# lucidrains/DALLE-pytorch

Measured on AMD Instinct MI355X. Metric: img-tokens/sec, higher is better.
Workload: dtype bf16; 1 GPU; model=dalle-dim1024-depth12-heads16, reversible=True, global_batch=64, seq_len=1280, image_seq_len=1024, parallelism=dp1, mode=train, eager=False

## Files before the change

dalle_pytorch_amd/ops/fp8.py:

```python

import weakref

import torch
import torch.nn.functional as F

from dalle_pytorch_amd.ops.dispatch import (env_flag, hip_module,
                                            using_eager_fallback)
from dalle_pytorch_amd.ops.fused import (fusion_enabled, geglu_bwd_colsum,
                                         geglu_colsum_tiles)

_FORCED = None
FP8_MAX = 448.0


def set_fp8_enabled(flag):
    global _FORCED
    _FORCED = bool(flag) if flag is not None else None


def fp8_enabled():
    if _FORCED is not None:
        return _FORCED
    return env_flag('FP8', False)


_generation = 0


def fp8_mark_step():
    global _generation
    _generation += 1


class _StepCache:

    BOUND = 512

    def __init__(self, make):
        self.make = make
        self.entries = {}

    def __call__(self, w):
        key = (w.data_ptr(), tuple(w.shape))
        stamp = (w._version, _generation)
        owner = w._base if w._base is not None else w
        hit = self.entries.get(key)
        if hit is not None and hit[0] == stamp and hit[2]() is owner:
            return hit[1]
        val = self.make(w)
        if len(self.entries) >= self.BOUND:
            self.entries.clear()
        self.entries[key] = (stamp, val, weakref.ref(owner))
        return val


def _bf16(w):
    w = w.detach()
    return w if w.dtype == torch.bfloat16 else w.to(torch.bfloat16)


def _quant(t, ext):
    t = t.detach().contiguous()
    scale = ext.amax_bf16(t)
    return ext.quant_fp8(t, scale), scale.squeeze()


_quant_weight = _StepCache(lambda w: _quant(_bf16(w), hip_module()))
_bf16_weight = _StepCache(_bf16)
_transposed_weight = _StepCache(lambda w: _bf16(w).t().contiguous())


def _fp8_ok(x, weight):
    if not fp8_enabled() or using_eager_fallback(x):
        return False
    if x.dtype != torch.bfloat16:
        return False
    rows = x.numel() // x.shape[-1]
    k, n = weight.shape[1], weight.shape[0]
    if rows % 16 or k % 16 or n % 16 or rows < 256:
        return False
    if rows * k < (32 << 20):
        return False
    return n * 2 >= k * 3


def _fast_dgrad_ok(x, w):
    if using_eager_fallback(x) or x.dtype != torch.bfloat16:
        return False
    rows = x.numel() // x.shape[-1]
    return (rows >= 1024 and rows % 16 == 0 and w.shape[0] % 16 == 0
            and w.shape[1] % 16 == 0 and torch.is_grad_enabled())


def _gemm_forward(x, weight, bias):
    x2 = x.reshape(-1, x.shape[-1])
    if _fp8_ok(x, weight):
        xq, xs = _quant(x2, hip_module())
        wq, ws = _quant_weight(weight)
        out = torch._scaled_mm(xq, wq.t(), scale_a=xs, scale_b=ws,
                               bias=bias, out_dtype=torch.bfloat16)
    else:
        wb = weight if weight.dtype == torch.bfloat16 else _bf16_weight(weight)
        out = F.linear(x, wb, bias).reshape(-1, weight.shape[0])
    return x2, out


def _gemm_backward(do2, x2, weight, lead):
    wt = _transposed_weight(weight)
    dx = (do2 @ wt.t()).reshape(*lead, weight.shape[1])
    dw = do2.t() @ x2.to(do2.dtype)
    return dx, dw.to(weight.dtype)


def _bf16_bias(bias):
    if bias is None or bias.dtype == torch.bfloat16:
        return bias
    return bias.to(torch.bfloat16)


class _LinearFn(torch.autograd.Function):

    @staticmethod
    def forward(ctx, x, weight, bias):
        x2, out = _gemm_forward(x, weight, _bf16_bias(bias))
        ctx.save_for_backward(x2, weight)
        ctx.has_bias = bias is not None
        return out.reshape(*x.shape[:-1], weight.shape[0])

    @staticmethod
    def backward(ctx, dout):
        x2, weight = ctx.saved_tensors
        do2 = dout.reshape(-1, dout.shape[-1]).contiguous()
        dx, dw = _gemm_backward(do2, x2, weight, dout.shape[:-1])
        return dx, dw, do2.sum(0) if ctx.has_bias else None


def fp8_linear_raw(x, weight, bias, module=None):
    if (_fp8_ok(x, weight) or _fast_dgrad_ok(x, weight)) \
            and weight.is_contiguous():
        return _LinearFn.apply(x.contiguous(), weight, bias)
    return F.linear(x, weight, bias) if module is None else module(x)


def fp8_linear(linear_module, x):
    return fp8_linear_raw(x, linear_module.weight, linear_module.bias,
                          linear_module)


class _LinearGegluFn(torch.autograd.Function):

    @staticmethod
    def forward(ctx, x, weight, bias):
        x2, h = _gemm_forward(x, weight, _bf16_bias(bias))
        out = hip_module().geglu_fwd(h)
        ctx.save_for_backward(x2, weight, h)
        ctx.bias_dtype = bias.dtype
        return out.reshape(*x.shape[:-1], weight.shape[0] // 2)

    @staticmethod
    def backward(ctx, dout):
        x2, weight, h = ctx.saved_tensors
        do2 = dout.reshape(-1, dout.shape[-1]).contiguous()
        dh, db = geglu_bwd_colsum(h, do2)
        dx, dw = _gemm_backward(dh, x2, weight, dout.shape[:-1])
        return dx, dw, db.to(ctx.bias_dtype)


def linear_geglu_ok(linear_module, x):
    w = linear_module.weight
    return (fusion_enabled('FF1_BIAS') and linear_module.bias is not None
            and (_fp8_ok(x, w) or _fast_dgrad_ok(x, w))
            and geglu_colsum_tiles(w.shape[0]))


def linear_geglu(linear_module, x):
    return _LinearGegluFn.apply(x.contiguous(), linear_module.weight,
                                linear_module.bias)
```

dalle_pytorch_amd/ops/hip/build.py:

```python

import os
import subprocess
import sys
import sysconfig
import time
from concurrent.futures import ThreadPoolExecutor
from pathlib import Path

PKG_DIR = Path(__file__).resolve().parents[2]
SRC_DIR = Path(__file__).resolve().parent
SOURCES = [SRC_DIR / name for name in (
    'attention.hip', 'decode.hip', 'train_ops.hip', 'module.hip')]
OBJ_DIR = SRC_DIR / 'build'
OUTPUT = PKG_DIR / '_hip.so'
MAX_JOBS = 16


def _mtime(path):
    return path.stat().st_mtime if path.exists() else 0.0


def toolchain():
    import torch
    from torch.utils import cpp_extension as ce

    hipcc = str(Path(ce.ROCM_HOME or '/opt/rocm') / 'bin' / 'hipcc')
    abi = '1' if torch._C._GLIBCXX_USE_CXX11_ABI else '0'
    inc = [f'-I{p}' for p in ce.include_paths()]
    inc.append(f"-I{sysconfig.get_paths()['include']}")
    flags = [
        '-O3', '-std=c++17', '--offload-arch=gfx950',
        '-fPIC',
        '-DTORCH_EXTENSION_NAME=_hip',
        '-DTORCH_API_INCLUDE_EXTENSION_H',
        f'-D_GLIBCXX_USE_CXX11_ABI={abi}',
        *ce.COMMON_HIP_FLAGS, *ce.COMMON_HIPCC_FLAGS,
        '-DTORCH_HIP_VERSION=' + torch.version.hip.split('.')[0],
        '-Wno-deprecated-declarations', '-Wno-unused-result',
        *inc,
    ]
    return hipcc, flags, [f'-L{p}' for p in ce.library_paths()]


def build(verbose=True, force=False):
    newest_hdr = max((_mtime(h) for h in SRC_DIR.glob('*.h')), default=0.0)
    newest_src = max(newest_hdr, *(_mtime(s) for s in SOURCES))
    if not force and _mtime(OUTPUT) > newest_src:
        if verbose:
            print(f'[build] {OUTPUT.name} up to date')
        return str(OUTPUT)
    objs = [OBJ_DIR / (s.stem + '.o') for s in SOURCES]
    stale = [(s, o) for s, o in zip(SOURCES, objs)
             if force or _mtime(o) <= max(_mtime(s), newest_hdr)]

    hipcc, flags, libdirs = toolchain()

    def compile_unit(pair):
        src, obj = pair
        tmp = obj.with_suffix('.tmp.o')
        cmd = [hipcc, *flags, '-c', str(src), '-o', str(tmp)]
        if verbose:
            print('[build]', ' '.join(cmd), flush=True)
        t0 = time.time()
        res = subprocess.run(cmd, stdout=subprocess.PIPE,
                             stderr=subprocess.STDOUT, text=True)
        if res.returncode == 0:
            tmp.replace(obj)
        return src.name, res, time.time() - t0

    if stale:
        OBJ_DIR.mkdir(exist_ok=True)
        jobs = min(len(stale), MAX_JOBS, os.cpu_count() or 1)
        with ThreadPoolExecutor(max_workers=jobs) as pool:
            results = list(pool.map(compile_unit, stale))
        for name, res, secs in results:
            if verbose or res.returncode != 0:
                print(f'[build] {name}: exit {res.returncode}, {secs:.0f} s\n'
                      f'{res.stdout}', end='', flush=True)
        failed = [name for name, res, _ in results if res.returncode != 0]
        if failed:
            raise RuntimeError('hipcc failed for ' + ', '.join(failed))

    cmd = [
        hipcc, '--offload-arch=gfx950', '-fPIC', '-shared',
        *[str(o) for o in objs], *libdirs,
        '-ltorch', '-ltorch_cpu', '-ltorch_hip', '-lc10', '-lc10_hip',
        '-ltorch_python', '-lamdhip64',
        '-o', str(OUTPUT),
    ]
    if verbose:
        print('[build]', ' '.join(cmd), flush=True)
    subprocess.run(cmd, check=True)
    return str(OUTPUT)


if __name__ == '__main__':
    build(force='--force' in sys.argv)
```

Measured before the change: 305,400 img_tokens_per_sec.

## Add split-K weight-gradient GEMM with fp32 partials and fused reduce kernel

Adds a split-K path for the linear-layer weight gradient. The long row dimension (tokens) is cut into S power-of-two chunks and run as a batched GEMM into fp32 partials. A custom HIP kernel then sums the partials and casts them to the weight dtype. The aim is to fill the GPU's many compute units when the weight's n×k output has too few tiles for the GEMM to use them all. The cost is extra memory traffic and workspace for the S fp32 partial matrices, plus one more kernel launch per linear backward.

```diff
diff --git a/dalle_pytorch_amd/ops/fp8.py b/dalle_pytorch_amd/ops/fp8.py
--- a/dalle_pytorch_amd/ops/fp8.py
+++ b/dalle_pytorch_amd/ops/fp8.py
@@ -105,11 +105,51 @@
     return x2, out
 
 
+WGRAD_TILE = 256
+WGRAD_TILE_TARGET = 192
+WGRAD_ROW_FLOOR = 16384
+WGRAD_CHUNK_FLOOR = 5120
+WGRAD_MAX_SPLITS = 32
+
+
+def wgrad_splits(rows, n, k):
+    if rows < WGRAD_ROW_FLOOR or n <= 0 or k <= 0 or n % 16 or k % 16:
+        return 1
+    tiles = -(-n // WGRAD_TILE) * -(-k // WGRAD_TILE)
+    s = 1
+    while (s * tiles < WGRAD_TILE_TARGET and s < WGRAD_MAX_SPLITS
+           and rows % (2 * s) == 0 and rows // (2 * s) >= WGRAD_CHUNK_FLOOR):
+        s *= 2
+    return s
+
+
+def wgrad_plan(do2, x2, out_dtype):
+    s = wgrad_splits(do2.shape[0], do2.shape[-1], x2.shape[-1])
+    if s <= 1:
+        return 0
+    if not fusion_enabled('WGRAD_SPLITK') or using_eager_fallback(do2):
+        return 0
+    if not (do2.dtype == x2.dtype == torch.bfloat16 and do2.dim() == 2
+            and x2.dim() == 2 and do2.is_contiguous() and x2.is_contiguous()
+            and out_dtype in (torch.float32, torch.bfloat16)):
+        return 0
+    return s
+
+
+def _wgrad_op(do2, x2, splits, out_dtype):
+    return torch.ops.dalle_amd.wgrad_splitk(do2, x2, splits, out_dtype)
+
+
 def _gemm_backward(do2, x2, weight, lead):
     wt = _transposed_weight(weight)
     dx = (do2 @ wt.t()).reshape(*lead, weight.shape[1])
-    dw = do2.t() @ x2.to(do2.dtype)
-    return dx, dw.to(weight.dtype)
+    x2 = x2.to(do2.dtype)
+    splits = wgrad_plan(do2, x2, weight.dtype)
+    if splits:
+        dw = _wgrad_op(do2, x2, splits, weight.dtype)
+    else:
+        dw = (do2.t() @ x2).to(weight.dtype)
+    return dx, dw
 
 
 def _bf16_bias(bias):
diff --git a/dalle_pytorch_amd/ops/hip/build.py b/dalle_pytorch_amd/ops/hip/build.py
--- a/dalle_pytorch_amd/ops/hip/build.py
+++ b/dalle_pytorch_amd/ops/hip/build.py
@@ -10,7 +10,8 @@
 PKG_DIR = Path(__file__).resolve().parents[2]
 SRC_DIR = Path(__file__).resolve().parent
 SOURCES = [SRC_DIR / name for name in (
-    'attention.hip', 'decode.hip', 'train_ops.hip', 'module.hip')]
+    'attention.hip', 'decode.hip', 'train_ops.hip', 'wgrad.hip',
+    'module.hip')]
 OBJ_DIR = SRC_DIR / 'build'
 OUTPUT = PKG_DIR / '_hip.so'
 MAX_JOBS = 16
diff --git a/dalle_pytorch_amd/ops/hip/wgrad.hip b/dalle_pytorch_amd/ops/hip/wgrad.hip
--- /dev/null
+++ b/dalle_pytorch_amd/ops/hip/wgrad.hip
@@ -0,0 +1,120 @@
+
+#include <torch/library.h>
+
+#include "hip_host.h"
+
+
+template <int S, bool OUT_BF16>
+__global__ __launch_bounds__(256)
+void wgrad_reduce_kernel(const f32x4* __restrict__ part,
+                         void* __restrict__ out,
+                         long nvec) {
+  for (long i = (long)blockIdx.x * 256 + threadIdx.x; i < nvec;
+       i += (long)gridDim.x * 256) {
+    f32x4 v[S];
+    #pragma unroll
+    for (int s = 0; s < S; ++s) v[s] = part[(long)s * nvec + i];
+    f32x4 acc = v[0];
+    #pragma unroll
+    for (int s = 1; s < S; ++s) acc += v[s];
+    if (OUT_BF16) {
+      bf16x4 o;
+      #pragma unroll
+      for (int e = 0; e < 4; ++e) o[e] = f2bf(acc[e]);
+      reinterpret_cast<bf16x4*>(out)[i] = o;
+    } else {
+      reinterpret_cast<f32x4*>(out)[i] = acc;
+    }
+  }
+}
+
+constexpr int WGRAD_MAX_SPLITS = 32;
+
+static bool wgrad_dtype_ok(at::ScalarType t) {
+  return t == at::kFloat || t == at::kBFloat16;
+}
+
+template <int S>
+static void launch_reduce(const torch::Tensor& part, torch::Tensor& out) {
+  const long nvec = out.numel() / 4;
+  const long nb = std::max<long>(std::min<long>((nvec + 255) / 256, 2048), 1);
+  auto* p = reinterpret_cast<const f32x4*>(part.data_ptr<float>());
+  if (out.scalar_type() == at::kBFloat16)
+    hipLaunchKernelGGL((wgrad_reduce_kernel<S, true>), dim3(nb), dim3(256), 0,
+                       cur_stream(), p, out.data_ptr(), nvec);
+  else
+    hipLaunchKernelGGL((wgrad_reduce_kernel<S, false>), dim3(nb), dim3(256),
+                       0, cur_stream(), p, out.data_ptr(), nvec);
+}
+
+torch::Tensor wgrad_reduce(const torch::Tensor& part,
+                           at::ScalarType out_dtype) {
+  TORCH_CHECK(part.is_cuda() && part.dim() == 3 && part.is_contiguous(),
+              "wgrad_reduce: partials must be a contiguous [S, n, k] GPU "
+              "tensor");
+  TORCH_CHECK(part.scalar_type() == at::kFloat && wgrad_dtype_ok(out_dtype),
+              "wgrad_reduce: partials must be float32, the output float32 or "
+              "bfloat16");
+  const long S = part.size(0), n = part.size(1), k = part.size(2);
+  TORCH_CHECK(n * k > 0 && (n * k) % 4 == 0,
+              "wgrad_reduce: n * k must be a positive multiple of 4, got ", n,
+              " x ", k);
+  auto out = at::empty({n, k}, part.options().dtype(out_dtype));
+  switch (S) {
+    case 1: launch_reduce<1>(part, out); break;
+    case 2: launch_reduce<2>(part, out); break;
+    case 4: launch_reduce<4>(part, out); break;
+    case 8: launch_reduce<8>(part, out); break;
+    case 16: launch_reduce<16>(part, out); break;
+    case 32: launch_reduce<32>(part, out); break;
+    default:
+      TORCH_CHECK(false, "wgrad_reduce: S must be a power of two <= ",
+                  WGRAD_MAX_SPLITS, ", got ", S);
+  }
+  return out;
+}
+
+torch::Tensor wgrad_splitk(const torch::Tensor& do2, const torch::Tensor& x2,
+                           int64_t splits, at::ScalarType out_dtype) {
+  TORCH_CHECK(do2.scalar_type() == at::kBFloat16 &&
+                  x2.scalar_type() == at::kBFloat16,
+              "wgrad_splitk: inputs must be bfloat16, got ",
+              do2.scalar_type(), " and ", x2.scalar_type());
+  TORCH_CHECK(do2.dim() == 2 && x2.dim() == 2,
+              "wgrad_splitk: inputs must be 2-D [rows, n] and [rows, k]");
+  TORCH_CHECK(do2.is_contiguous() && x2.is_contiguous(),
+              "wgrad_splitk: inputs must be contiguous");
+  TORCH_CHECK(do2.size(0) == x2.size(0),
+              "wgrad_splitk: row counts differ: ", do2.size(0), " vs ",
+              x2.size(0));
+  TORCH_CHECK(wgrad_dtype_ok(out_dtype),
+              "wgrad_splitk: out_dtype must be float32 or bfloat16");
+  const long M = do2.size(0), n = do2.size(1), k = x2.size(1);
+  const long S = splits;
+  TORCH_CHECK(S >= 1 && S <= WGRAD_MAX_SPLITS && (S & (S - 1)) == 0,
+              "wgrad_splitk: splits must be a power of two <= ",
+              WGRAD_MAX_SPLITS, ", got ", S);
+  TORCH_CHECK(M > 0 && M % S == 0, "wgrad_splitk: splits = ", S,
+              " does not divide the ", M, " rows");
+  TORCH_CHECK(n * k > 0 && (n * k) % 4 == 0,
+              "wgrad_splitk: n * k must be a positive multiple of 4, got ", n,
+              " x ", k);
+  TORCH_CHECK(do2.is_cuda() && x2.is_cuda() &&
+                  do2.device() == x2.device(),
+              "wgrad_splitk: inputs must be GPU tensors on one device");
+  auto a = do2.view({S, M / S, n}).transpose(1, 2);
+  auto b = x2.view({S, M / S, k});
+  auto part = at::empty({S, n, k}, do2.options().dtype(at::kFloat));
+  at::bmm_out(part, a, b, at::kFloat);
+  if (S == 1 && out_dtype == at::kFloat) return part.view({n, k});
+  return wgrad_reduce(part, out_dtype);
+}
+
+#ifndef __HIP_DEVICE_COMPILE__
+TORCH_LIBRARY(dalle_amd, m) {
+  m.def("wgrad_splitk(Tensor do2, Tensor x2, int splits, "
+        "ScalarType out_dtype) -> Tensor", &wgrad_splitk);
+  m.def("wgrad_reduce(Tensor part, ScalarType out_dtype) -> Tensor",
+        &wgrad_reduce);
+}
+#endif
```

Result: faster. 316,000 img_tokens_per_sec (median of 6 runs) (+3.5%).
